# prachigarg23/MDIL-SS

Hardware: AMD Instinct MI355X
Metric: images/sec at 1024x512 ERFNet-RA step-2 train (CS->BDD, KD on), batch 6/GPU (higher is better)
Workload: dtype f32; 1 GPU; ERFNet-RAP step-2 (2 student fwd + teacher fwd + CE + 0.1*KLD + bwd + Adam), random-init weights of the reference architecture, num_classes [20,20]; batch_per_gpu=6, global_batch=6, height=512, width=1024, parallelism=dp1

## Files before the change

### include/mdil_hip.h

```cpp
#ifndef MDIL_HIP_H
#define MDIL_HIP_H

#include <stddef.h>

#ifdef __cplusplus
extern "C" {
#endif

#define MDIL_OK 0
#define MDIL_ERR_INVALID (-1)
#define MDIL_ERR_LAUNCH (-2)
#define MDIL_ERR_UNSUPPORTED (-3)

#define MDIL_MAX_TAPS 9

const char* mdil_last_error(void);
int mdil_version(void);

typedef struct mdil_geom {
  int N, HO, WO;
  int HI, WI;
  int ihs, iws;
  int ntaps;
  int dh[MDIL_MAX_TAPS], dw[MDIL_MAX_TAPS];
  int src[MDIL_MAX_TAPS];
  int in_pitch[2];
  int OH, OW;
  int ohs, oho, ows, owo;
  int out_pitch, out_coff;
} mdil_geom;

typedef struct mdil_epilogue {
  const float* bias;
  const float* scale;
  const float* shift;
  const float* res;
  const float* res_gate;
  const float* gate;
  int relu;
  const float* bias2;
} mdil_epilogue;

typedef struct mdil_pack_job {
  const float* src;
  float* dst;
  int ntaps, M, K, M_P, K_P, s_m, s_k, stem;
  int ktap[MDIL_MAX_TAPS];
} mdil_pack_job;
int mdil_pack_weights(const float* src, float* dst, int ntaps, const int* ktap, int M, int K,
                      int M_P, int K_P, int s_m, int s_k, int stem, void* stream);
int mdil_pack_weights_batch(const mdil_pack_job* jobs_device, int njobs, void* stream);

int mdil_tapconv(const mdil_geom* g, int cin, int cout, const float* in0, const float* in1,
                 const float* wpk, const mdil_epilogue* epi, float* out, void* stream);

int mdil_tapconv_stat_blocks(const mdil_geom* g, int cin, int cout);
int mdil_tapconv_stats(const mdil_geom* g, int cin, int cout, const float* in0, const float* in1,
                       const float* wpk, const mdil_epilogue* epi, float* out, float* partial,
                       float* pcount, void* stream);


typedef struct mdil_bn_train {
  const float *gamma, *beta;
  float *running_mean, *running_var;
  long long* num_batches_tracked;
  float eps, momentum;
  float* coef;
} mdil_bn_train;
int mdil_tapconv_bn_train(const mdil_geom* g, int cin, int cout, const float* in0, const float* in1,
                          const float* wpk, const mdil_epilogue* epi, float* out,
                          const mdil_bn_train* bn, void* workspace, size_t workspace_bytes,
                          unsigned int* ticket, void* stream);

typedef struct mdil_bn_grad {
  const float* gamma;
  float *dgamma, *dbeta;
  int accumulate;
  float* coef;
  unsigned int* ticket;
} mdil_bn_grad;

int mdil_tapconv_bnred(const mdil_geom* g, int cin, int cout, const float* in0, const float* in1,
                       const float* wpk, const mdil_epilogue* epi, float* out, const float* bn_z,
                       const float* save_mean, const float* save_invstd, float* partial,
                       const mdil_bn_grad* fin, void* stream);

typedef struct mdil_bn_tail {
  const float* gate;
  const float* z;
  const float* save_mean;
  const float* save_invstd;
  const float* drop;
  float* partial;
  mdil_bn_grad fin;
} mdil_bn_tail;
int mdil_tapconv_tail_blocks(const mdil_geom* g, int cin, int cout);
int mdil_tapconv_tail(const mdil_geom* g, int cin, int cout, const float* in0, const float* in1,
                      const float* wpk, const mdil_epilogue* epi, float* out, const mdil_bn_tail* tail,
                      void* stream);

size_t mdil_wgrad_workspace(const mdil_geom* g, int cin, int cout);
int mdil_wgrad(const mdil_geom* g, int cin, int cout, const float* in0, const float* in1,
               const float* gout, const int* ktap, int s_co, int s_ci, float* dw, float* dbias,
               int ntaps2, int s_co2, int s_ci2, float* dw2, float* dbias2,
               int accumulate ,
               void* workspace, size_t workspace_bytes, void* stream);

// ... 135 lines not shown
```

### mdil_ss_amd/_lib.py

```python
import ctypes as C
import os

_HERE = os.path.dirname(os.path.abspath(__file__))
LIB_PATH = os.environ.get("MDIL_HIP_LIB", os.path.join(_HERE, "libmdil_hip.so"))
MAX_TAPS = 9


class Geom(C.Structure):
    _fields_ = [("N", C.c_int), ("HO", C.c_int), ("WO", C.c_int), ("HI", C.c_int), ("WI", C.c_int),
                ("ihs", C.c_int), ("iws", C.c_int), ("ntaps", C.c_int),
                ("dh", C.c_int * MAX_TAPS), ("dw", C.c_int * MAX_TAPS), ("src", C.c_int * MAX_TAPS),
                ("in_pitch", C.c_int * 2), ("OH", C.c_int), ("OW", C.c_int),
                ("ohs", C.c_int), ("oho", C.c_int), ("ows", C.c_int), ("owo", C.c_int),
                ("out_pitch", C.c_int), ("out_coff", C.c_int)]


class PackJob(C.Structure):
    _fields_ = [("src", C.c_void_p), ("dst", C.c_void_p), ("ntaps", C.c_int), ("M", C.c_int),
                ("K", C.c_int), ("M_P", C.c_int), ("K_P", C.c_int), ("s_m", C.c_int),
                ("s_k", C.c_int), ("stem", C.c_int), ("ktap", C.c_int * MAX_TAPS)]


class Epilogue(C.Structure):
    _fields_ = [("bias", C.c_void_p), ("scale", C.c_void_p), ("shift", C.c_void_p),
# ... 8 lines not shown
        "dbeta")]


class BnGrad(C.Structure):
    _fields_ = [("gamma", C.c_void_p), ("dgamma", C.c_void_p), ("dbeta", C.c_void_p),
                ("accumulate", C.c_int), ("coef", C.c_void_p), ("ticket", C.c_void_p)]


class BnTrain(C.Structure):
    _fields_ = [("gamma", C.c_void_p), ("beta", C.c_void_p), ("running_mean", C.c_void_p),
                ("running_var", C.c_void_p), ("num_batches_tracked", C.c_void_p),
                ("eps", C.c_float), ("momentum", C.c_float), ("coef", C.c_void_p)]


class BnTail(C.Structure):
    _fields_ = [(n, C.c_void_p) for n in ("gate", "z", "save_mean", "save_invstd", "drop", "partial")] + \
               [("fin", BnGrad)]


class NbBlock(C.Structure):
    _fields_ = [("N", C.c_int), ("H", C.c_int), ("W", C.c_int), ("C", C.c_int),
                ("dilation", C.c_int), ("rap", C.c_int), ("train", C.c_int),
                ("bn_eps", C.c_float), ("bn_momentum", C.c_float), ("half", NbHalf * 2)] + \
               [(n, C.c_void_p) for n in ("x", "drop", "a1", "z1", "u", "a2", "z2", "out", "gy",
                                          "gz2", "ga", "gu", "gx")] + \
               [("bn_workspace", C.c_void_p), ("bn_workspace_bytes", C.c_size_t),
                ("wgrad_workspace", C.c_void_p), ("wgrad_workspace_bytes", C.c_size_t),
                ("head_partial", C.c_void_p), ("head_nblk", C.c_int), ("tail", BnTail),
                ("head_coef", C.c_void_p), ("ticket", C.c_void_p), ("eval_coef_ready", C.c_int)]


class WgradJob(C.Structure):
    _fields_ = [("opaque", C.c_ubyte * 192)]


class ProfileRecord(C.Structure):
    _fields_ = [("kind", C.c_int), ("path", C.c_int), ("cin", C.c_int), ("cout", C.c_int),
                ("ntaps", C.c_int), ("npix", C.c_longlong), ("ms", C.c_float)]


_P = C.c_void_p
_I = C.c_int
_L = C.c_longlong
_F = C.c_float
_D = C.c_double
_Z = C.c_size_t

_SIGNATURES = {
    "mdil_last_error": (C.c_char_p, []),
    "mdil_version": (_I, []),
    "mdil_pack_weights": (_I, [_P, _P, _I, C.POINTER(_I), _I, _I, _I, _I, _I, _I, _I, _P]),
    "mdil_pack_weights_batch": (_I, [_P, _I, _P]),
    "mdil_tapconv": (_I, [C.POINTER(Geom), _I, _I, _P, _P, _P, C.POINTER(Epilogue), _P, _P]),
    "mdil_tapconv_stat_blocks": (_I, [C.POINTER(Geom), _I, _I]),
    "mdil_tapconv_stats": (_I, [C.POINTER(Geom), _I, _I, _P, _P, _P, C.POINTER(Epilogue), _P, _P, _P, _P]),
    "mdil_tapconv_bnred": (_I, [C.POINTER(Geom), _I, _I, _P, _P, _P, C.POINTER(Epilogue), _P, _P, _P, _P,
                                _P, C.POINTER(BnGrad), _P]),
    "mdil_tapconv_bn_train": (_I, [C.POINTER(Geom), _I, _I, _P, _P, _P, C.POINTER(Epilogue), _P,
                                   C.POINTER(BnTrain), _P, _Z, _P, _P]),
    "mdil_bn_backward_apply": (_I, [_P, _P, _P, _L, _I, _I, _P, _P, _P, _P, _P]),
    "mdil_tapconv_tail_blocks": (_I, [C.POINTER(Geom), _I, _I]),
    "mdil_tapconv_tail": (_I, [C.POINTER(Geom), _I, _I, _P, _P, _P, C.POINTER(Epilogue), _P,
                               C.POINTER(BnTail), _P]),
    "mdil_nb_block_tail_blocks": (_I, [_I, _I, _I, _I, _I]),
    "mdil_bn_backward_partials": (_I, [_P, _P, _P, _L, _I, _I, _P, _P, _P, _P, _I, _P, _P, _I, _P, _P, _Z, _P]),
    "mdil_bn_train_finalize": (_I, [_P, _P, _I, _I, _P, _P, _P, _P, _P, _F, _F, _P, _P, _P, _P, _P]),
    "mdil_wgrad_workspace": (_Z, [C.POINTER(Geom), _I, _I]),
    "mdil_wgrad": (_I, [C.POINTER(Geom), _I, _I, _P, _P, _P, C.POINTER(_I), _I, _I, _P, _P,
                   _I, _I, _I, _P, _P, _I, _P, _Z, _P]),
    "mdil_bn_workspace": (_Z, [_L, _I]),
    "mdil_bn_train_stats": (_I, [_P, _L, _I, _P, _P, _P, _P, _P, _F, _F, _P, _P, _P, _P, _P, _Z, _P, _P]),
    "mdil_bn_eval_coeffs": (_I, [_I, _P, _P, _P, _P, _F, _P, _P, _P]),
    "mdil_bn_apply": (_I, [_P, _L, _I, _I, _P, _P, _P, _P, _I, _P, _P]),
    "mdil_bn_backward": (_I, [_P, _P, _P, _P, _L, _I, _I, _P, _P, _P, _P, _P, _I, _P, _P, _Z, _P, _P]),
    "mdil_maxpool_concat_fwd": (_I, [_P, _I, _I, _I, _I, _P, _I, _I, _P]),
    "mdil_maxpool_concat_bwd": (_I, [_P, _P, _I, _I, _I, _I, _I, _I, _P, _P]),
    "mdil_outconv_fwd": (_I, [_P, _P, _P, _I, _I, _I, _I, _I, _P, _P]),
    "mdil_nb_block_wgrad_workspace": (_Z, [_I, _I, _I, _I, _I, _I]),
    "mdil_nb_block_forward": (_I, [C.POINTER(NbBlock), _P]),
    "mdil_nb_block_backward": (_I, [C.POINTER(NbBlock), _P]),
    "mdil_nb_block_backward_deferred": (_I, [C.POINTER(NbBlock), C.POINTER(WgradJob), C.POINTER(_I),
                                             C.POINTER(_Z), _P]),
    "mdil_wgrad_deferred": (_I, [C.POINTER(Geom), _I, _I, _P, _P, _P, C.POINTER(_I), _I, _I, _P, _P,
                            _I, _I, _I, _P, _P, _P, _Z, C.POINTER(WgradJob), _P]),
    "mdil_wgrad_reduce_batch": (_I, [C.POINTER(WgradJob), _I, _P]),
    "mdil_head_workspace": (_Z, []),
    "mdil_head_ce": (_I, [_P, _P, _P, _I, _I, _I, _I, _P, _P, _P, _P, _P, _P, _P, _P, _I, _P, _P, _P, _Z, _P]),
    "mdil_head_kld": (_I, [_P, _P, _P, _P, _P, _P, _I, _I, _I, _I, _P, _P, _P, _P, _P, _I, _P, _Z, _P]),
    "mdil_loss_workspace": (_Z, [_L]),
    "mdil_ce_loss": (_I, [_P, _P, _P, _L, _I, _I, _P, _P, _P, _P, _P, _Z, _P]),
    "mdil_kld_loss": (_I, [_P, _P, _L, _I, _I, _P, _P, _P, _P, _Z, _P]),
    "mdil_argmax_confusion": (_I, [_P, _P, _L, _I, _I, _I, _P, _P, _P]),
    "mdil_adam_step": (_I, [_P, _P, _P, _P, _L, _D, _D, _D, _D, _D, _D, _D, _D, _P]),
    "mdil_augment_batch": (_I, [_P, _P, _P, _I, _I, _I, _I, _I, _P, _P, _P]),
    "mdil_nchw_to_nhwc": (_I, [_P, _I, _I, _I, _I, _P, _P]),
    "mdil_dropout_factors": (_I, [_P, _P, _P, _P, _I, _P]),
    "mdil_profile_begin": (_I, [_I]),
    "mdil_profile_end": (_I, [C.POINTER(ProfileRecord), _I]),
}

EXPORTS = tuple(_SIGNATURES)
_lib = None


def load():
    global _lib
# ... 21 lines not shown
```

### mdil_ss_amd/ops.py

```python
import ctypes as C
import weakref as _weakref

import torch

from . import _lib
from ._lib import Epilogue, Geom

BN_EPS = 1e-3
BN_MOMENTUM = 0.1


_raw_stream = torch._C._cuda_getCurrentRawStream
_cur_device = torch._C._cuda_getDevice


def _stream():
    return _raw_stream(_cur_device())


def _p(t):
    return None if t is None else t.data_ptr()


def _chk(t, name="tensor"):
# ... 563 lines not shown
    return gz


def bn_backward_partials(g, z, gamma, beta, coef, want_affine, partial, nblk, out=None):
    lib = _lib.load()
    Cc = z.shape[-1]
    npix = z.numel() // Cc
    gz = torch.empty_like(z) if out is None else out
    dg = db = None
    sunk = False
    if want_affine:
        sg, sb = _sink(gamma), _sink(beta)
        sunk = sg is not None and sb is not None
        if sunk:
            dg, db = sg, sb
        else:
            dgb = torch.zeros(2, Cc, dtype=torch.float32, device=z.device)
            dg, db = dgb[0], dgb[1]
    ws = _bn_ws(lib, npix, Cc, z.device)
    cws = ws.data_ptr() + (256 * 2 * Cc + 256) * 4
    _lib.check(lib.mdil_bn_backward_partials(_p(g), None, _p(z), npix, npix // z.shape[0], Cc, _p(gamma),
                                             coef.data_ptr(), coef.data_ptr() + 4 * Cc, partial, nblk,
                                             _p(dg), _p(db), 1, _p(gz), cws, 3 * Cc * 4, _stream()),
               "mdil_bn_backward_partials")
    if sunk or not want_affine:
        return gz, None, None
    return gz, dg, db


def _g_s1(N, H, W, Cc, taps, two_src=False):
    return make_geom(N, H, W, H, W, taps, Cc, H, W, Cc)


def _taps_3x1(d, flip=False):
    s = -1 if flip else 1
    return [(s * (k - 1) * d, 0, 0) for k in range(3)]


def _taps_1x3(d, flip=False):
    s = -1 if flip else 1
    return [(0, s * (k - 1) * d, 0) for k in range(3)]


_PAR = {0: [(1, 0)], 1: [(0, 1), (2, 0)]}


def _class_taps(a, b):
    taps, ktap = [], []
    for kh, dh in _PAR[a]:
        for kw, dw in _PAR[b]:
            taps.append((dh, dw, 0))
            ktap.append(kh * 3 + kw)
    return taps, ktap


class DownFn(torch.autograd.Function):

    @staticmethod
    def forward(ctx, x, w, b, gamma, beta, rm, rv, nbt, train, link_out):
        lib = _lib.load()
        ctx.sink_slot = SINK_SLOT
        ctx.link_out = link_out
        _chk(x, "x")
        N, H, W, cin = x.shape
        cc = w.shape[0]
        cout = cc + cin
        HO, WO = H // 2, W // 2
        stem = cin == 3
        z = torch.empty(N, HO, WO, cout, dtype=torch.float32, device=x.device)
        if stem:
            wp = _cached((w.data_ptr(), "stem"), lambda: pack_into(
                torch.empty(1, 16, 32, dtype=torch.float32, device=w.device), w, (0,), cc, 27,
                27, 1, stem=True), (w,))
            g = make_geom(N, HO, WO, H, W, [(0, 0, 0)], 3, HO, WO, cout, ihs=2, iws=2)
            tapconv(g, 27, cc, x, None, wp, z, bias=b)
        else:
            taps = [(kh - 1, kw - 1, 0) for kh in range(3) for kw in range(3)]
            g = make_geom(N, HO, WO, H, W, taps, cin, HO, WO, cout, ihs=2, iws=2)
            tapconv(g, cin, cc, x, None, pack_conv(w, "fwd"), z, bias=b)
        _lib.check(lib.mdil_maxpool_concat_fwd(_p(x), N, H, W, cin, _p(z), cout, cc, _stream()),
                   "mdil_maxpool_concat_fwd")
        if train:
            coef = bn_train_stats(z, gamma, beta, rm, rv, nbt)
            y = bn_apply(z, coef[2], coef[3], relu=True)
            ctx.save_for_backward(x, w, b, gamma, beta, z, y, coef)
            _log_gates(y)
            _attach_tail(link_out, y, z, coef, gamma, beta)
        else:
            ec = bn_eval_coeffs(gamma, beta, rm, rv)
            y = bn_apply(z, ec[0], ec[1], relu=True)
        ctx.stem = stem
        return y

    @staticmethod
    def backward(ctx, gy):
        global SINK_SLOT
        SINK_SLOT = ctx.sink_slot
        lib = _lib.load()
        x, w, b, gamma, beta, z, y, coef = ctx.saved_tensors
        gy = gy.contiguous()
        N, H, W, cin = x.shape
        cc = w.shape[0]
        cout = cc + cin
        HO, WO = H // 2, W // 2
        need = ctx.needs_input_grad
        gz, dgamma, dbeta = _bn_backward_maybe_fused(ctx.link_out, gy, y, z, gamma, beta, coef, need[3] or need[4])
        dw = db = gx = None
        if need[1] or need[2]:
            if ctx.stem:
                g = make_geom(N, HO, WO, H, W, [(0, 0, 0)], 3, HO, WO, cout, ihs=2, iws=2)
                dw, db = wgrad(g, 27, cc, x, None, gz, None, 0, 0, w, b)
            else:
                taps = [(kh - 1, kw - 1, 0) for kh in range(3) for kw in range(3)]
                g = make_geom(N, HO, WO, H, W, taps, cin, HO, WO, cout, ihs=2, iws=2)
                dw, db = wgrad(g, cin, cc, x, None, gz, tuple(range(9)), cin * 9, 9, w, b)
        if need[0]:
            gx = torch.empty_like(x)
            _lib.check(lib.mdil_maxpool_concat_bwd(_p(x), _p(gz), N, H, W, cin, cout, cc, _p(gx),
                                                   _stream()), "mdil_maxpool_concat_bwd")
            for a in (0, 1):
                for bb in (0, 1):
                    taps, ktap = _class_taps(a, bb)
                    g = make_geom(N, HO, WO, HO, WO, taps, cout, H, W, cin, ohs=2, oho=a, ows=2,
                                  owo=bb)
                    tapconv(g, cc, cin, gz, None, pack_conv(w, "dgrad", tuple(ktap)), gx, res=gx)
        return gx, dw, db, dgamma, dbeta, None, None, None, None, None


def _pack_pair_dgrad(w31, pw):
    if pw is None:
        return pack_conv(w31, "dgrad")
    Cc = w31.shape[0]

    def build():
        dst = torch.empty(4, Cc, Cc, dtype=torch.float32, device=w31.device)
        pack_into(dst[:3], w31, (0, 1, 2), Cc, Cc, 3, Cc * 3)
        pack_into(dst[3:], pw, (0,), Cc, Cc, 1, Cc)
        return dst

    return _cached((w31.data_ptr(), pw.data_ptr(), "pair_dgrad"), build, (w31, pw))


BLOCK_ABI = __import__("os").environ.get("MDIL_PY_BLOCKS") is None
_nb_ws_bytes = {}


DEFER_WGRAD = False
WGRAD_BATCH = int(__import__("os").environ.get("MDIL_WGRAD_BATCH", "16"))
WGRAD_ARENA_BYTES = WGRAD_BATCH * (20 << 20)


class _DeferState:
    __slots__ = ("jobs", "n", "cursor", "arena", "nout", "used")

    def __init__(self, device):
        self.jobs = (_lib.WgradJob * (WGRAD_BATCH + 4))()
        self.n = 0
        self.cursor = 0
        self.arena = torch.empty(WGRAD_ARENA_BYTES, dtype=torch.uint8, device=device)
        self.nout = C.c_int(0)
        self.used = C.c_size_t(0)


_defer_states = {}


def _defer_state(device):
    key = (_cur_device(), _raw_stream(_cur_device()))
    st = _defer_states.get(key)
    if st is None:
        if torch.cuda.is_current_stream_capturing():
            raise RuntimeError("mdil: the weight-gradient arena would be allocated during graph capture; "
                               "run one eager iteration on the same streams first")
        st = _defer_states[key] = _DeferState(device)
    return st


def flush_wgrad():
# ... 350 lines not shown
                    dw13, db13 = conv_wgrad(_taps_1x3(dil), a, gz, w13, b13)
                if pw is not None and npw:
                    dpw, dpb = conv_wgrad([(0, 0, 0)], inp, gz, pw, pb)
            G = make_geom(N, H, W, H, W, _taps_1x3(dil, flip=True), Cc, H, W, Cc)
            ga = tapconv(G, Cc, Cc, gz, None, pack_conv(w13, "dgrad"), torch.empty_like(gz), gate=a)
            if n31:
                dw31, db31 = conv_wgrad(_taps_3x1(dil), inp, ga, w31, b31)
            taps = _taps_3x1(dil, flip=True)
            wpk = _pack_pair_dgrad(w31, pw)
            if pw is not None:
                taps = taps + [(0, 0, 1)]
            G = make_geom(N, H, W, H, W, taps, Cc, H, W, Cc)
            fused = None
            if bnred is not None and res_in is None and not BN_BWD_UNFUSED:
                fused = tapconv_bnred(G, Cc, Cc, ga, gz, wpk, torch.empty_like(gz), *bnred)
            if fused is not None:
                ginp = fused
            else:
                ginp = tapconv(G, Cc, Cc, ga, gz, wpk, torch.empty_like(gz), res=res_in,
                               res_gate=res_gate)
            return ginp, dw31, db31, dw13, db13, dpw, dpb

        gz2, dg2, dbe2 = bn_backward(gy, out, drop, z2, g2, be2, c2, need[15] or need[16])
        gu, dw31_2, db31_2, dw13_2, db13_2, dpw2, dpb2 = pair_bwd(
            gz2, a2, u, w31_2, b31_2, w13_2, b13_2, pw2, pb2, ctx.dil, need[9] or need[10], need[11] or need[12],
            need[13] or need[14], None, None, bnred=(u, z1, c1))
        if isinstance(gu, tuple):
            g_, partial, nblk = gu
            gz1, dg1, dbe1 = bn_backward_partials(g_, z1, g1, be1, c1, need[7] or need[8], partial,
                                                  nblk, out=g_)
        else:
            gz1, dg1, dbe1 = bn_backward(gu, u, None, z1, g1, be1, c1, need[7] or need[8], out=gu)
        gx, dw31_1, db31_1, dw13_1, db13_1, dpw1, dpb1 = pair_bwd(
            gz1, a1, x, w31_1, b31_1, w13_1, b13_1, pw1, pb1, 1, need[1] or need[2], need[3] or need[4],
            need[5] or need[6], gy, out)
        res = [gx, dw31_1, db31_1, dw13_1, db13_1, dpw1, dpb1, dg1, dbe1,
               dw31_2, db31_2, dw13_2, db13_2, dpw2, dpb2, dg2, dbe2, None, None, None, None, None, None]
        for i in range(17):
            if not need[i]:
                res[i] = None
        return tuple(res)


class UpFn(torch.autograd.Function):

    @staticmethod
    def forward(ctx, x, w, b, gamma, beta, rm, rv, nbt, train, link_out):
        ctx.sink_slot = SINK_SLOT
        ctx.link_out = link_out
        _chk(x, "x")
        N, H, W, cin = x.shape
        cout = w.shape[1]
        z = torch.empty(N, 2 * H, 2 * W, cout, dtype=torch.float32, device=x.device)
        for a in (0, 1):
            for bb in (0, 1):
                taps, ktap = _class_taps(a, bb)
                g = make_geom(N, H, W, H, W, taps, cin, 2 * H, 2 * W, cout, ohs=2, oho=a, ows=2,
                              owo=bb)
                tapconv(g, cin, cout, x, None, pack_conv(w, "t_fwd", tuple(ktap)), z, bias=b)
        if train:
            coef = bn_train_stats(z, gamma, beta, rm, rv, nbt)
            y = bn_apply(z, coef[2], coef[3], relu=True)
            ctx.save_for_backward(x, w, b, gamma, beta, z, y, coef)
            _log_gates(y)
            _attach_tail(link_out, y, z, coef, gamma, beta)
        else:
            ec = bn_eval_coeffs(gamma, beta, rm, rv)
            y = bn_apply(z, ec[0], ec[1], relu=True, out=z)
        return y

    @staticmethod
    def backward(ctx, gy):
        global SINK_SLOT
        SINK_SLOT = ctx.sink_slot
        x, w, b, gamma, beta, z, y, coef = ctx.saved_tensors
        gy = gy.contiguous()
        N, H, W, cin = x.shape
        cout = w.shape[1]
        need = ctx.needs_input_grad
        gz, dgamma, dbeta = _bn_backward_maybe_fused(ctx.link_out, gy, y, z, gamma, beta, coef, need[3] or need[4])
        dw = db = gx = None
        if need[1] or need[2]:
            for a in (0, 1):
                for bb in (0, 1):
                    taps, ktap = _class_taps(a, bb)
                    g = make_geom(N, H, W, H, W, taps, cin, 2 * H, 2 * W, cout, ohs=2, oho=a, ows=2,
                                  owo=bb)
                    dw, db = wgrad(g, cin, cout, x, None, gz, tuple(ktap), 9, cout * 9, w, b, dw, db)
        if need[0]:
            taps = [(kh - 1, kw - 1, 0) for kh in range(3) for kw in range(3)]
            g = make_geom(N, H, W, 2 * H, 2 * W, taps, cout, H, W, cin, ihs=2, iws=2)
            gx = tapconv(g, cout, cin, gz, None, pack_conv(w, "t_dgrad"), torch.empty_like(x))
        return gx, dw, db, dgamma, dbeta, None, None, None, None, None


def _r4(v):
    return (v + 3) // 4 * 4


class OutFn(torch.autograd.Function):

    @staticmethod
    def forward(ctx, x, w, b):
        ctx.sink_slot = SINK_SLOT
        _chk(x, "x")
        N, H, W, cin = x.shape
        nc = w.shape[1]
        P = _r4(nc)
        y = torch.empty(N, 2 * H, 2 * W, P, dtype=torch.float32, device=x.device)
        if cin == 16 and w.is_contiguous() and b is not None:
            _lib.check(_lib.load().mdil_outconv_fwd(_p(x), _p(w), _p(b), N, H, W, nc, P, _p(y),
                                                    _stream()), "mdil_outconv_fwd")
# ... 346 lines not shown
```

Measured before the change: 271.6 images/sec.

## Merge four sub-pixel class convolutions into one kernel for upsample and downsample dgrad

Adds a HIP kernel that computes all four output parity classes of the stride-2 transposed-conv forward and the downsampler data-gradient in a single launch. Each input tile is loaded once and reused across the 3x3 taps, with MFMA accumulators for all four classes and interleaved output stores. The downsampler backward also folds the maxpool-concat gradient into the epilogue, which removes a separate kernel and the read-modify-write residual passes over gx. The cost is higher register and LDS pressure from keeping four accumulator sets, and only four fixed channel configurations are supported.

After: 274.3 images/sec (median of 6 runs). About the same (+1.0%).

```diff
diff --git a/include/mdil_hip.h b/include/mdil_hip.h
--- a/include/mdil_hip.h
+++ b/include/mdil_hip.h
@@ -53,6 +53,10 @@
 
 int mdil_tapconv(const mdil_geom* g, int cin, int cout, const float* in0, const float* in1,
                  const float* wpk, const mdil_epilogue* epi, float* out, void* stream);
+
+int mdil_tapconv_classes(int N, int H, int W, int cin, int cout, const float* in, int in_pitch,
+                         const float* wpk, const mdil_epilogue* epi, float* out, int out_pitch,
+                         const float* pool_x, int pool_coff, void* stream);
 
 int mdil_tapconv_stat_blocks(const mdil_geom* g, int cin, int cout);
 int mdil_tapconv_stats(const mdil_geom* g, int cin, int cout, const float* in0, const float* in1,
diff --git a/mdil_ss_amd/_lib.py b/mdil_ss_amd/_lib.py
--- a/mdil_ss_amd/_lib.py
+++ b/mdil_ss_amd/_lib.py
@@ -84,6 +84,7 @@
     "mdil_pack_weights": (_I, [_P, _P, _I, C.POINTER(_I), _I, _I, _I, _I, _I, _I, _I, _P]),
     "mdil_pack_weights_batch": (_I, [_P, _I, _P]),
     "mdil_tapconv": (_I, [C.POINTER(Geom), _I, _I, _P, _P, _P, C.POINTER(Epilogue), _P, _P]),
+    "mdil_tapconv_classes": (_I, [_I, _I, _I, _I, _I, _P, _I, _P, C.POINTER(Epilogue), _P, _I, _P, _I, _P]),
     "mdil_tapconv_stat_blocks": (_I, [C.POINTER(Geom), _I, _I]),
     "mdil_tapconv_stats": (_I, [C.POINTER(Geom), _I, _I, _P, _P, _P, C.POINTER(Epilogue), _P, _P, _P, _P]),
     "mdil_tapconv_bnred": (_I, [C.POINTER(Geom), _I, _I, _P, _P, _P, C.POINTER(Epilogue), _P, _P, _P, _P,
diff --git a/mdil_ss_amd/csrc/tapconv_classes.hip b/mdil_ss_amd/csrc/tapconv_classes.hip
--- /dev/null
+++ b/mdil_ss_amd/csrc/tapconv_classes.hip
@@ -0,0 +1,321 @@
+#include <type_traits>
+
+#include "common.h"
+
+namespace {
+
+constexpr int pos_dh(int p) { return p < 2 ? 1 : 0; }
+constexpr int pos_dw(int p) { return (p == 0 || p == 2) ? 1 : 0; }
+constexpr int pos_ntile(int p) { return p == 0 ? 1 : (p == 3 ? 4 : 2); }
+constexpr int pos_cls(int p, int j) { return p == 0 ? 3 : p == 1 ? (j == 0 ? 2 : 3) : p == 2 ? (j == 0 ? 1 : 3) : j; }
+constexpr int pos_tap(int p, int j) {
+  return p == 0 ? 0 : p == 1 ? (j == 0 ? 1 : 2) : p == 2 ? (j == 0 ? 3 : 6) : (j == 0 ? 4 : j == 1 ? 5 : j == 2 ? 7 : 8);
+}
+
+struct ClsArgs {
+  int N, H, W;
+  int in_pitch, out_pitch;
+  int pool_coff;
+  const float* in;
+  const float* wpk;
+  const float* pool_x;
+  float* out;
+};
+
+template <int CIN, int COUT, int BM_>
+struct ClsCfg {
+  static constexpr int BM = BM_;
+  static constexpr int KC = (CIN <= 48) ? CIN : 32;
+  static constexpr int NCHUNK = CIN / KC;
+  static constexpr int QPR = KC / 4;
+  static constexpr int LD = KC + 4;
+  static constexpr int MT = COUT / 16;
+  static constexpr int NT = BM / 16;
+  static constexpr bool SPLIT_CO = (MT % 4 == 0);
+  static constexpr int TM = SPLIT_CO ? MT / 4 : MT;
+  static constexpr int TN = SPLIT_CO ? NT : NT / 4;
+  static constexpr int IN_ITEMS = BM * QPR / MDIL_WG;
+  static constexpr int W_ITEMS = (COUT * QPR + MDIL_WG - 1) / MDIL_WG;
+  static constexpr int LDO = COUT + 4;
+  static constexpr int QO = COUT / 4;
+  static constexpr int SMEM_STAGE = (BM + 4 * COUT) * LD;
+  static constexpr int SMEM_OUT = 2 * BM * LDO + 2 * BM;
+  static constexpr int SMEM = SMEM_STAGE > SMEM_OUT ? SMEM_STAGE : SMEM_OUT;
+  static_assert(CIN % 16 == 0 && COUT % 16 == 0, "channel counts");
+  static_assert(CIN % KC == 0, "chunking");
+  static_assert((BM * QPR) % MDIL_WG == 0, "in-tile items");
+  static_assert(SPLIT_CO || (NT % 4 == 0), "pixel tiles per wave");
+  static_assert(MDIL_WG % QO == 0 && (BM * 2 * QO) % MDIL_WG == 0, "store loop");
+  static_assert(BM <= MDIL_WG, "output offsets");
+};
+
+template <int CIN, int COUT, int BM, bool POOL>
+__global__ __launch_bounds__(MDIL_WG) void tapconv_classes_kernel(const ClsArgs A, const mdil_epilogue e) {
+  using C = ClsCfg<CIN, COUT, BM>;
+  __shared__ __attribute__((aligned(16))) float smem[C::SMEM];
+  float* Is = smem;
+  float* Ws = smem + BM * C::LD;
+
+  const int tid = threadIdx.x;
+  const int lane = tid & 63, wave = tid >> 6;
+  const int li = lane & 15, lg = lane >> 4;
+  const int hw = A.H * A.W;
+  const int npix = A.N * hw;
+  const int tile0 = blockIdx.x * BM;
+
+  int it_i[C::IN_ITEMS], it_j[C::IN_ITEMS];
+  long long it_base[C::IN_ITEMS];
+#pragma unroll
+  for (int i = 0; i < C::IN_ITEMS; ++i) {
+    const int idx = tid + MDIL_WG * i;
+    const int P = tile0 + idx / C::QPR;
+    if (P < npix) {
+      const int r = P % hw;
+      it_i[i] = r / A.W;
+      it_j[i] = r - it_i[i] * A.W;
+      it_base[i] = (long long)P * A.in_pitch;
+    } else {
+      it_i[i] = 1 << 28;
+      it_j[i] = 0;
+      it_base[i] = 0;
+    }
+  }
+
+  f32x4 regI[C::IN_ITEMS];
+  f32x4 regW[4][C::W_ITEMS];
+  unsigned okI = 0;
+
+  auto issue_loads = [&](auto POS, int kc) {
+    constexpr int p = decltype(POS)::value;
+    constexpr int dh = pos_dh(p), dw = pos_dw(p);
+    const long long tap_off = ((long long)dh * A.W + dw) * A.in_pitch + kc * C::KC;
+#pragma unroll
+    for (int i = 0; i < C::IN_ITEMS; ++i) {
+      const int q = (tid + MDIL_WG * i) % C::QPR;
+      const bool ok = (it_i[i] + dh < A.H) && (it_j[i] + dw < A.W);
+      long long off = it_base[i] + (q * 4 + tap_off);
+      off = ok ? off : 0ll;
+      regI[i] = *reinterpret_cast<const f32x4*>(A.in + off);
+      okI = ok ? (okI | (1u << i)) : (okI & ~(1u << i));
+    }
+#pragma unroll
+    for (int j = 0; j < pos_ntile(p); ++j) {
+#pragma unroll
+      for (int i = 0; i < C::W_ITEMS; ++i) {
+        int idx = tid + MDIL_WG * i;
+        if constexpr ((COUT * C::QPR) % MDIL_WG != 0) idx = idx < COUT * C::QPR ? idx : 0;
+        const int co = idx / C::QPR, q = idx % C::QPR;
+        regW[j][i] = *reinterpret_cast<const f32x4*>(A.wpk + ((long long)(pos_tap(p, j) * COUT + co)) * CIN +
+                                                     kc * C::KC + q * 4);
+      }
+    }
+  };
+
+  auto write_lds = [&](auto POS) {
+    constexpr int p = decltype(POS)::value;
+#pragma unroll
+    for (int i = 0; i < C::IN_ITEMS; ++i) {
+      const int idx = tid + MDIL_WG * i;
+      const int px = idx / C::QPR, q = idx % C::QPR;
+      const f32x4 z = {0.f, 0.f, 0.f, 0.f};
+      *reinterpret_cast<f32x4*>(&Is[px * C::LD + q * 4]) = ((okI >> i) & 1u) ? regI[i] : z;
+    }
+#pragma unroll
+    for (int j = 0; j < pos_ntile(p); ++j) {
+#pragma unroll
+      for (int i = 0; i < C::W_ITEMS; ++i) {
+        const int idx = tid + MDIL_WG * i;
+        if (((COUT * C::QPR) % MDIL_WG == 0) || idx < COUT * C::QPR) {
+          const int co = idx / C::QPR, q = idx % C::QPR;
+          *reinterpret_cast<f32x4*>(&Ws[(j * COUT + co) * C::LD + q * 4]) = regW[j][i];
+        }
+      }
+    }
+  };
+
+  f32x4 acc[4][C::TM][C::TN];
+#pragma unroll
+  for (int c = 0; c < 4; ++c)
+#pragma unroll
+    for (int m = 0; m < C::TM; ++m)
+#pragma unroll
+      for (int n = 0; n < C::TN; ++n) acc[c][m][n] = f32x4{0.f, 0.f, 0.f, 0.f};
+
+  const int co_tile0 = C::SPLIT_CO ? wave * C::TM : 0;
+  const int px_tile0 = C::SPLIT_CO ? 0 : wave * C::TN;
+
+  auto mfma_stage = [&](auto POS) {
+    constexpr int p = decltype(POS)::value;
+#pragma unroll
+    for (int r = 0; r < C::KC / 16; ++r) {
+      f32x4 b[C::TN];
+#pragma unroll
+      for (int n = 0; n < C::TN; ++n)
+        b[n] = *reinterpret_cast<const f32x4*>(&Is[((px_tile0 + n) * 16 + li) * C::LD + r * 16 + lg * 4]);
+#pragma unroll
+      for (int j = 0; j < pos_ntile(p); ++j) {
+        f32x4 a[C::TM];
+#pragma unroll
+        for (int m = 0; m < C::TM; ++m)
+          a[m] = *reinterpret_cast<const f32x4*>(
+              &Ws[(j * COUT + (co_tile0 + m) * 16 + li) * C::LD + r * 16 + lg * 4]);
+#pragma unroll
+        for (int s = 0; s < 4; ++s)
+#pragma unroll
+          for (int m = 0; m < C::TM; ++m)
+#pragma unroll
+            for (int n = 0; n < C::TN; ++n)
+              acc[pos_cls(p, j)][m][n] = mfma16(a[m][s], b[n][s], acc[pos_cls(p, j)][m][n]);
+      }
+    }
+  };
+
+  auto position = [&](auto POS) {
+    constexpr int p = decltype(POS)::value;
+    for (int kc = 0; kc < C::NCHUNK; ++kc) {
+      __syncthreads();
+      write_lds(POS);
+      __syncthreads();
+      if (kc + 1 < C::NCHUNK) {
+        issue_loads(POS, kc + 1);
+      } else if constexpr (p < 3) {
+        issue_loads(std::integral_constant<int, p + 1>{}, 0);
+      }
+      __builtin_amdgcn_s_setprio(1);
+      mfma_stage(POS);
+      __builtin_amdgcn_s_setprio(0);
+    }
+  };
+  issue_loads(std::integral_constant<int, 0>{}, 0);
+  position(std::integral_constant<int, 0>{});
+  position(std::integral_constant<int, 1>{});
+  position(std::integral_constant<int, 2>{});
+  position(std::integral_constant<int, 3>{});
+
+  float* Os = smem;
+  long long* Ob = reinterpret_cast<long long*>(smem + 2 * BM * C::LDO);
+  const int OW = 2 * A.W;
+  const int q4 = (tid % C::QO) * 4;
+  f32x4 vscale = {1.f, 1.f, 1.f, 1.f}, vbias = {0.f, 0.f, 0.f, 0.f};
+  if (e.bias) vbias = *reinterpret_cast<const f32x4*>(e.bias + q4);
+  if (e.bias2) vbias += *reinterpret_cast<const f32x4*>(e.bias2 + q4);
+  if (e.scale) {
+    vscale = *reinterpret_cast<const f32x4*>(e.scale + q4);
+    vbias = vbias * vscale + *reinterpret_cast<const f32x4*>(e.shift + q4);
+  }
+#pragma unroll
+  for (int a = 0; a < 2; ++a) {
+    __syncthreads();
+#pragma unroll
+    for (int b = 0; b < 2; ++b)
+#pragma unroll
+      for (int n = 0; n < C::TN; ++n)
+#pragma unroll
+        for (int m = 0; m < C::TM; ++m)
+          *reinterpret_cast<f32x4*>(
+              &Os[(((px_tile0 + n) * 16 + li) * 2 + b) * C::LDO + (co_tile0 + m) * 16 + lg * 4]) =
+              acc[a * 2 + b][m][n];
+    if (a == 0 && tid < BM) {
+      const int P = tile0 + tid;
+      long long ob = -1;
+      if (P < npix) {
+        const int ni = P / hw;
+        const int r = P - ni * hw;
+        const int i = r / A.W;
+        const int j = r - i * A.W;
+        ob = ((long long)(ni * 2 * A.H + 2 * i) * OW + 2 * j) * A.out_pitch;
+      }
+      Ob[tid] = ob;
+    }
+    __syncthreads();
+    constexpr int NIT = BM * 2 * C::QO / MDIL_WG;
+#pragma unroll
+    for (int it = 0; it < NIT; ++it) {
+      const int idx = tid + it * MDIL_WG;
+      const int px = idx / (2 * C::QO);
+      const int b = (idx / C::QO) & 1;
+      const long long ob = Ob[px];
+      const bool ok = ob >= 0;
+      const long long obase = ok ? ob + ((long long)a * OW + b) * A.out_pitch + q4 : 0ll;
+      f32x4 v = *reinterpret_cast<const f32x4*>(&Os[(px * 2 + b) * C::LDO + q4]);
+      v = v * vscale + vbias;
+      if constexpr (POOL) {
+        const long long wb = ok ? ob + q4 : 0ll;
+        const long long down = (long long)OW * A.out_pitch;
+        const f32x4 x0 = *reinterpret_cast<const f32x4*>(A.pool_x + wb);
+        const f32x4 x1 = *reinterpret_cast<const f32x4*>(A.pool_x + wb + (ok ? A.out_pitch : 0));
+        const f32x4 x2 = *reinterpret_cast<const f32x4*>(A.pool_x + wb + (ok ? down : 0ll));
+        const f32x4 x3 = *reinterpret_cast<const f32x4*>(A.pool_x + wb + (ok ? down + A.out_pitch : 0ll));
+        const long long goff = ok ? (long long)(tile0 + px) * A.in_pitch + A.pool_coff + q4 : 0ll;
+        const f32x4 gg = *reinterpret_cast<const f32x4*>(A.in + goff);
+        f32x4 rr;
+#pragma unroll
+        for (int k = 0; k < 4; ++k) {
+          float m = x0[k];
+          int arg = 0;
+          if (x1[k] > m) { m = x1[k]; arg = 1; }
+          if (x2[k] > m) { m = x2[k]; arg = 2; }
+          if (x3[k] > m) { m = x3[k]; arg = 3; }
+          rr[k] = arg == a * 2 + b ? gg[k] : 0.f;
+        }
+        v += rr;
+      }
+      if (e.relu) {
+#pragma unroll
+        for (int k = 0; k < 4; ++k) v[k] = fmaxf(v[k], 0.f);
+      }
+      if (ok) __builtin_nontemporal_store(v, reinterpret_cast<f32x4*>(A.out + obase));
+    }
+  }
+}
+
+template <int CIN, int COUT, int BM>
+int launch_classes(const ClsArgs& a, const mdil_epilogue* epi, hipStream_t st) {
+  const long long npix = (long long)a.N * a.H * a.W;
+  const int grid = cdiv(npix, BM);
+  if (a.pool_x)
+    hipLaunchKernelGGL((tapconv_classes_kernel<CIN, COUT, BM, true>), dim3(grid), dim3(MDIL_WG), 0, st, a, *epi);
+  else
+    hipLaunchKernelGGL((tapconv_classes_kernel<CIN, COUT, BM, false>), dim3(grid), dim3(MDIL_WG), 0, st, a, *epi);
+  MDIL_CHECK_LAUNCH();
+  return MDIL_OK;
+}
+
+}
+
+extern "C" int mdil_tapconv_classes(int N, int H, int W, int cin, int cout, const float* in, int in_pitch,
+                                    const float* wpk, const mdil_epilogue* epi, float* out, int out_pitch,
+                                    const float* pool_x, int pool_coff, void* stream) {
+  MDIL_CHECK_ARG(in && wpk && epi && out, "tapconv_classes: null argument");
+  if (!((cin == 128 && cout == 64) || (cin == 64 && cout == 16) || (cin == 64 && cout == 64) ||
+        (cin == 48 && cout == 16))) {
+    mdil_set_error("tapconv_classes: no tile configuration for cin=%d cout=%d", cin, cout);
+    return MDIL_ERR_UNSUPPORTED;
+  }
+  MDIL_CHECK_ARG(N >= 1 && H >= 1 && W >= 1, "tapconv_classes: empty grid");
+  MDIL_CHECK_ARG((long long)N * H * W * 4 < (1ll << 31), "tapconv_classes: grid too large");
+  MDIL_CHECK_ARG(in_pitch >= cin && in_pitch % 4 == 0, "tapconv_classes: in_pitch=%d", in_pitch);
+  MDIL_CHECK_ARG(out_pitch >= cout && out_pitch % 4 == 0, "tapconv_classes: out_pitch=%d", out_pitch);
+  MDIL_CHECK_ARG((epi->scale == nullptr) == (epi->shift == nullptr), "tapconv_classes: scale/shift");
+  MDIL_CHECK_ARG(!epi->res && !epi->res_gate && !epi->gate, "tapconv_classes: residual / gate epilogues");
+  MDIL_CHECK_ARG(!pool_x || (pool_coff >= 0 && pool_coff % 4 == 0 && pool_coff + cout <= in_pitch),
+                 "tapconv_classes: pool_coff=%d", pool_coff);
+  ClsArgs a;
+  a.N = N, a.H = H, a.W = W;
+  a.in_pitch = in_pitch, a.out_pitch = out_pitch, a.pool_coff = pool_coff;
+  a.in = in, a.wpk = wpk, a.pool_x = pool_x, a.out = out;
+  hipStream_t st = (hipStream_t)stream;
+  mdil_geom g;
+  memset(&g, 0, sizeof(g));
+  g.N = N, g.HO = H, g.WO = W, g.ntaps = 9;
+  MdilProfScope ps(st, 0, &g, cin, cout);
+#define CL(ci, co, bm) \
+  if (cin == ci && cout == co) return launch_classes<ci, co, bm>(a, epi, st)
+  CL(128, 64, 64);
+  CL(64, 16, 128);
+  CL(64, 64, 64);
+  CL(48, 16, 128);
+#undef CL
+  mdil_set_error("tapconv_classes: no tile configuration for cin=%d cout=%d", cin, cout);
+  return MDIL_ERR_UNSUPPORTED;
+}
diff --git a/mdil_ss_amd/ops.py b/mdil_ss_amd/ops.py
--- a/mdil_ss_amd/ops.py
+++ b/mdil_ss_amd/ops.py
@@ -639,6 +639,19 @@
             taps.append((dh, dw, 0))
             ktap.append(kh * 3 + kw)
     return taps, ktap
+
+
+CLASS_MERGED = __import__("os").environ.get("MDIL_NO_CLSCONV") is None
+
+
+def tapconv_classes(x, cin, cout, wpk, out, bias=None, scale=None, shift=None, relu=False, pool_x=None,
+                    pool_coff=0):
+    N, H, W, pitch = x.shape
+    e = Epilogue(_p(bias), _p(scale), _p(shift), None, None, None, 1 if relu else 0, None)
+    _lib.check(_lib.load().mdil_tapconv_classes(N, H, W, cin, cout, _p(x), pitch, _p(wpk), C.byref(e),
+                                                _p(out), out.shape[3], _p(pool_x), pool_coff, _stream()),
+               "mdil_tapconv_classes")
+    return out
 
 
 class DownFn(torch.autograd.Function):
@@ -703,14 +716,17 @@
                 dw, db = wgrad(g, cin, cc, x, None, gz, tuple(range(9)), cin * 9, 9, w, b)
         if need[0]:
             gx = torch.empty_like(x)
-            _lib.check(lib.mdil_maxpool_concat_bwd(_p(x), _p(gz), N, H, W, cin, cout, cc, _p(gx),
-                                                   _stream()), "mdil_maxpool_concat_bwd")
-            for a in (0, 1):
-                for bb in (0, 1):
-                    taps, ktap = _class_taps(a, bb)
-                    g = make_geom(N, HO, WO, HO, WO, taps, cout, H, W, cin, ohs=2, oho=a, ows=2,
-                                  owo=bb)
-                    tapconv(g, cc, cin, gz, None, pack_conv(w, "dgrad", tuple(ktap)), gx, res=gx)
+            if CLASS_MERGED:
+                tapconv_classes(gz, cc, cin, pack_conv(w, "dgrad"), gx, pool_x=x, pool_coff=cc)
+            else:
+                _lib.check(lib.mdil_maxpool_concat_bwd(_p(x), _p(gz), N, H, W, cin, cout, cc, _p(gx),
+                                                       _stream()), "mdil_maxpool_concat_bwd")
+                for a in (0, 1):
+                    for bb in (0, 1):
+                        taps, ktap = _class_taps(a, bb)
+                        g = make_geom(N, HO, WO, HO, WO, taps, cout, H, W, cin, ohs=2, oho=a, ows=2,
+                                      owo=bb)
+                        tapconv(g, cc, cin, gz, None, pack_conv(w, "dgrad", tuple(ktap)), gx, res=gx)
         return gx, dw, db, dgamma, dbeta, None, None, None, None, None
 
 
@@ -1167,12 +1183,15 @@
         N, H, W, cin = x.shape
         cout = w.shape[1]
         z = torch.empty(N, 2 * H, 2 * W, cout, dtype=torch.float32, device=x.device)
-        for a in (0, 1):
-            for bb in (0, 1):
-                taps, ktap = _class_taps(a, bb)
-                g = make_geom(N, H, W, H, W, taps, cin, 2 * H, 2 * W, cout, ohs=2, oho=a, ows=2,
-                              owo=bb)
-                tapconv(g, cin, cout, x, None, pack_conv(w, "t_fwd", tuple(ktap)), z, bias=b)
+        if CLASS_MERGED:
+            tapconv_classes(x, cin, cout, pack_conv(w, "t_fwd"), z, bias=b)
+        else:
+            for a in (0, 1):
+                for bb in (0, 1):
+                    taps, ktap = _class_taps(a, bb)
+                    g = make_geom(N, H, W, H, W, taps, cin, 2 * H, 2 * W, cout, ohs=2, oho=a, ows=2,
+                                  owo=bb)
+                    tapconv(g, cin, cout, x, None, pack_conv(w, "t_fwd", tuple(ktap)), z, bias=b)
         if train:
             coef = bn_train_stats(z, gamma, beta, rm, rv, nbt)
             y = bn_apply(z, coef[2], coef[3], relu=True)
```

## Fuse four stride-2 parity-class tap convolutions into one kernel sharing input tiles

Applied to the files above, without the earlier changes.

Adds a HIP kernel that computes all four output parity classes of a stride-2 transposed convolution (upsample forward and downsample input-gradient) in a single launch. It loads one shared 2x2-shifted input tile into LDS and runs MFMA over all nine taps, instead of four separate tapconv launches that each re-read the input. It uses persistent work-groups capped at twice the CU count and falls back to the old path for uncovered shapes. Coverage is limited to a few specific channel configurations, and the fixed tiling may lower occupancy.

Measured after the change: 270.6 images/sec before, 271.4 images/sec after, median of 6. No clear change (+0.3%).

```diff
diff --git a/include/mdil_hip.h b/include/mdil_hip.h
--- a/include/mdil_hip.h
+++ b/include/mdil_hip.h
@@ -53,6 +53,10 @@
 
 int mdil_tapconv(const mdil_geom* g, int cin, int cout, const float* in0, const float* in1,
                  const float* wpk, const mdil_epilogue* epi, float* out, void* stream);
+
+int mdil_tapconv_s2x4_covers(const mdil_geom* g, int cin, int cout, const mdil_epilogue* epi);
+int mdil_tapconv_s2x4(const mdil_geom* g, int cin, int cout, const float* in0, const float* wpk9,
+                      const mdil_epilogue* epi, float* out, void* stream);
 
 int mdil_tapconv_stat_blocks(const mdil_geom* g, int cin, int cout);
 int mdil_tapconv_stats(const mdil_geom* g, int cin, int cout, const float* in0, const float* in1,
diff --git a/mdil_ss_amd/_lib.py b/mdil_ss_amd/_lib.py
--- a/mdil_ss_amd/_lib.py
+++ b/mdil_ss_amd/_lib.py
@@ -84,6 +84,8 @@
     "mdil_pack_weights": (_I, [_P, _P, _I, C.POINTER(_I), _I, _I, _I, _I, _I, _I, _I, _P]),
     "mdil_pack_weights_batch": (_I, [_P, _I, _P]),
     "mdil_tapconv": (_I, [C.POINTER(Geom), _I, _I, _P, _P, _P, C.POINTER(Epilogue), _P, _P]),
+    "mdil_tapconv_s2x4_covers": (_I, [C.POINTER(Geom), _I, _I, C.POINTER(Epilogue)]),
+    "mdil_tapconv_s2x4": (_I, [C.POINTER(Geom), _I, _I, _P, _P, C.POINTER(Epilogue), _P, _P]),
     "mdil_tapconv_stat_blocks": (_I, [C.POINTER(Geom), _I, _I]),
     "mdil_tapconv_stats": (_I, [C.POINTER(Geom), _I, _I, _P, _P, _P, C.POINTER(Epilogue), _P, _P, _P, _P]),
     "mdil_tapconv_bnred": (_I, [C.POINTER(Geom), _I, _I, _P, _P, _P, C.POINTER(Epilogue), _P, _P, _P, _P,
diff --git a/mdil_ss_amd/csrc/tapconv4.hip b/mdil_ss_amd/csrc/tapconv4.hip
--- /dev/null
+++ b/mdil_ss_amd/csrc/tapconv4.hip
@@ -0,0 +1,285 @@
+#include <stdlib.h>
+
+#include "common.h"
+
+namespace {
+
+__host__ __device__ constexpr int tap_cls(int t) { return t == 0 ? 0 : t < 3 ? 1 : t < 5 ? 2 : 3; }
+__host__ __device__ constexpr int tap_shift(int t) {
+  return (int)(((1u << 2 | 2u << 6 | 3u << 10 | 2u << 12 | 1u << 14) >> (2 * t)) & 3u);
+}
+
+template <int CIN, int COUT, int BM_, int KC_>
+struct X4Cfg {
+  static constexpr int BM = BM_, KC = KC_;
+  static constexpr int CIN_P = CIN;
+  static constexpr int NCH = CIN_P / KC;
+  static constexpr int QPR = KC / 4;
+  static constexpr int LD = KC + 4;
+  static constexpr int MT = COUT / 16, COUT_P = COUT;
+  static constexpr int NT = BM / 16;
+  static constexpr bool SPLIT_CO = (MT == 4);
+  static constexpr int TM = 1;
+  static constexpr int TN = SPLIT_CO ? NT : 1;
+  static constexpr int IN_ROWS = 4 * BM, W_ROWS = 9 * COUT_P;
+  static constexpr int IN_ITEMS = IN_ROWS * QPR / MDIL_WG;
+  static constexpr int W_ITEMS = (W_ROWS * QPR + MDIL_WG - 1) / MDIL_WG;
+  static constexpr bool W_RAGGED = (W_ROWS * QPR) % MDIL_WG != 0;
+  static constexpr int SMEM_STAGE = (IN_ROWS + W_ROWS) * LD;
+  static constexpr int LDO = COUT + 4;
+  static constexpr int SMEM_EPI_MAX = (NCH == 1) ? IN_ROWS * LD : SMEM_STAGE;
+  static constexpr int EPASS = (4 * BM * LDO + 2 * BM <= SMEM_EPI_MAX) ? 1 : 2;
+  static constexpr int CPP = 4 / EPASS;
+  static constexpr int QO = COUT / 4;
+  static constexpr int NIT = CPP * BM * QO / MDIL_WG;
+  static_assert(CIN % 16 == 0 && COUT % 16 == 0 && CIN_P % KC == 0 && KC % 16 == 0, "channels");
+  static_assert((IN_ROWS * QPR) % MDIL_WG == 0, "in-tile items");
+  static_assert(SPLIT_CO || (MT == 1 && NT == 2), "wave split");
+  static_assert(CPP * BM * LDO + 2 * BM <= SMEM_EPI_MAX, "epilogue staging");
+  static_assert((CPP * BM * QO) % MDIL_WG == 0 && MDIL_WG % QO == 0, "store items");
+  static_assert(SMEM_STAGE * 4 <= 80 * 1024, "two work-groups per CU");
+};
+
+template <int CIN, int COUT, int BM, int KC>
+__global__ __launch_bounds__(MDIL_WG) void tapconv4_kernel(const mdil_geom g, const float* __restrict__ in0,
+                                                           const float* __restrict__ wpk,
+                                                           const float* __restrict__ bias, const float* res,
+                                                           float* out) {
+  using C = X4Cfg<CIN, COUT, BM, KC>;
+  __shared__ __attribute__((aligned(16))) float smem[C::SMEM_STAGE];
+  float* Is = smem;
+  float* Ws = smem + C::IN_ROWS * C::LD;
+
+  const int tid = threadIdx.x;
+  const int lane = tid & 63;
+  const int wave = __builtin_amdgcn_readfirstlane(tid >> 6);
+  const int li = lane & 15, lg = lane >> 4;
+  const int npix = g.N * g.HO * g.WO;
+  const int hw = g.HO * g.WO;
+  const int pitch = g.in_pitch[0];
+  const int ntile = (npix + BM - 1) / BM;
+  const int my_tiles = ((int)blockIdx.x < ntile) ? (ntile - 1 - (int)blockIdx.x) / (int)gridDim.x + 1 : 0;
+  const int nstage = my_tiles * C::NCH;
+
+  const int co_tile0 = C::SPLIT_CO ? wave : 0;
+  const int px_tile0 = C::SPLIT_CO ? 0 : (wave & 1);
+  const unsigned cls_mask = C::SPLIT_CO ? 0xFu : ((wave >> 1) ? 0x6u : 0x9u);
+
+  long long it_off[C::IN_ITEMS];
+  f32x4 regI[C::IN_ITEMS];
+  f32x4 regW[C::W_ITEMS];
+
+  auto issue_loads = [&](int st) {
+    const int tile = blockIdx.x + (st / C::NCH) * gridDim.x;
+    const int kc = st % C::NCH;
+    if (kc == 0) {
+#pragma unroll
+      for (int i = 0; i < C::IN_ITEMS; ++i) {
+        const int row = (tid + MDIL_WG * i) / C::QPR;
+        const int s = row / BM, p = row % BM;
+        const int P = tile * BM + p;
+        long long off = -1;
+        if (P < npix) {
+          const int n = P / hw;
+          const int r = P - n * hw;
+          const int h = r / g.WO;
+          const int hi = h + (s >> 1), wi = r - h * g.WO + (s & 1);
+          if (hi < g.HI && wi < g.WI) off = (((long long)n * g.HI + hi) * g.WI + wi) * pitch;
+        }
+        it_off[i] = off;
+      }
+    }
+#pragma unroll
+    for (int i = 0; i < C::IN_ITEMS; ++i) {
+      const int q = (tid + MDIL_WG * i) % C::QPR;
+      const long long off = it_off[i] < 0 ? 0ll : it_off[i];
+      regI[i] = *reinterpret_cast<const f32x4*>(in0 + off + kc * KC + q * 4);
+    }
+    if (C::NCH > 1 || st == 0) {
+#pragma unroll
+      for (int i = 0; i < C::W_ITEMS; ++i) {
+        int idx = tid + MDIL_WG * i;
+        if constexpr (C::W_RAGGED) idx = idx < C::W_ROWS * C::QPR ? idx : 0;
+        const int row = idx / C::QPR, q = idx % C::QPR;
+        regW[i] = *reinterpret_cast<const f32x4*>(wpk + (long long)row * C::CIN_P + kc * KC + q * 4);
+      }
+    }
+  };
+
+  auto write_lds = [&](int st) {
+#pragma unroll
+    for (int i = 0; i < C::IN_ITEMS; ++i) {
+      const int idx = tid + MDIL_WG * i;
+      const int row = idx / C::QPR, q = idx % C::QPR;
+      const f32x4 z = {0.f, 0.f, 0.f, 0.f};
+      *reinterpret_cast<f32x4*>(&Is[row * C::LD + q * 4]) = it_off[i] < 0 ? z : regI[i];
+    }
+    if (C::NCH > 1 || st == 0) {
+#pragma unroll
+      for (int i = 0; i < C::W_ITEMS; ++i) {
+        const int idx = tid + MDIL_WG * i;
+        if (!C::W_RAGGED || idx < C::W_ROWS * C::QPR) {
+          const int row = idx / C::QPR, q = idx % C::QPR;
+          *reinterpret_cast<f32x4*>(&Ws[row * C::LD + q * 4]) = regW[i];
+        }
+      }
+    }
+  };
+
+  f32x4 acc[4][C::TN];
+  auto zero_acc = [&]() {
+#pragma unroll
+    for (int c = 0; c < 4; ++c)
+#pragma unroll
+      for (int n = 0; n < C::TN; ++n) acc[c][n] = f32x4{0.f, 0.f, 0.f, 0.f};
+  };
+  zero_acc();
+
+  f32x4 vbias = {0.f, 0.f, 0.f, 0.f};
+  if (bias) vbias = *reinterpret_cast<const f32x4*>(bias + (tid % C::QO) * 4);
+
+  auto epilogue = [&](int tile) {
+    float* Os = smem;
+    long long* Ob = reinterpret_cast<long long*>(smem + C::CPP * BM * C::LDO);
+#pragma unroll
+    for (int pass = 0; pass < C::EPASS; ++pass) {
+      __syncthreads();
+#pragma unroll
+      for (int c = 0; c < C::CPP; ++c) {
+        const int cls = pass * C::CPP + c;
+        if ((cls_mask >> cls) & 1u) {
+          const int a_local = c >> 1, b = c & 1;
+#pragma unroll
+          for (int n = 0; n < C::TN; ++n) {
+            const int p = (px_tile0 + n) * 16 + li;
+            *reinterpret_cast<f32x4*>(&Os[((a_local * BM + p) * 2 + b) * C::LDO + co_tile0 * 16 + lg * 4]) =
+                acc[cls][n];
+          }
+        }
+      }
+      if (pass == 0 && tid < BM) {
+        const int P = tile * BM + tid;
+        long long ob = -1;
+        if (P < npix) {
+          const int n = P / hw;
+          const int r = P - n * hw;
+          const int h = r / g.WO;
+          const int w = r - h * g.WO;
+          ob = (((long long)n * g.OH + 2 * h) * g.OW + 2 * w) * g.out_pitch + g.out_coff;
+        }
+        Ob[tid] = ob;
+      }
+      __syncthreads();
+#pragma unroll
+      for (int it = 0; it < C::NIT; ++it) {
+        const int idx = tid + it * MDIL_WG;
+        const int row = idx / C::QO, q = idx % C::QO;
+        const int b = row & 1, p = (row >> 1) % BM;
+        const int a = (C::EPASS == 2) ? pass : (row >> 1) / BM;
+        const long long ob = Ob[p];
+        const bool ok = ob >= 0;
+        const long long o = (ok ? ob : 0ll) + ((long long)a * g.OW + b) * g.out_pitch + q * 4;
+        f32x4 v = *reinterpret_cast<const f32x4*>(&Os[row * C::LDO + q * 4]);
+        v = v + vbias;
+        if (res) v += *reinterpret_cast<const f32x4*>(res + (ok ? o : 0ll));
+        if (ok) __builtin_nontemporal_store(v, reinterpret_cast<f32x4*>(out + o));
+      }
+    }
+  };
+
+  if (nstage > 0) issue_loads(0);
+  for (int st = 0; st < nstage; ++st) {
+    __syncthreads();
+    write_lds(st);
+    __syncthreads();
+    if (st + 1 < nstage) issue_loads(st + 1);
+    __builtin_amdgcn_s_setprio(1);
+#pragma unroll
+    for (int t = 0; t < 9; ++t) {
+      const int cls = tap_cls(t), sh = tap_shift(t);
+      if ((cls_mask >> cls) & 1u) {
+#pragma unroll
+        for (int r = 0; r < KC / 16; ++r) {
+          f32x4 b[C::TN];
+          const f32x4 a =
+              *reinterpret_cast<const f32x4*>(&Ws[((t * C::MT + co_tile0) * 16 + li) * C::LD + r * 16 + lg * 4]);
+#pragma unroll
+          for (int n = 0; n < C::TN; ++n)
+            b[n] = *reinterpret_cast<const f32x4*>(
+                &Is[(sh * BM + (px_tile0 + n) * 16 + li) * C::LD + r * 16 + lg * 4]);
+#pragma unroll
+          for (int s = 0; s < 4; ++s)
+#pragma unroll
+            for (int n = 0; n < C::TN; ++n) acc[cls][n] = mfma16(a[s], b[n][s], acc[cls][n]);
+        }
+      }
+    }
+    __builtin_amdgcn_s_setprio(0);
+    if (st % C::NCH == C::NCH - 1) {
+      epilogue(blockIdx.x + (st / C::NCH) * gridDim.x);
+      zero_acc();
+    }
+  }
+}
+
+int x4_num_cu() {
+  static int n_cu = 0;
+  if (n_cu == 0) {
+    int dev = 0, n = 0;
+    if (hipGetDevice(&dev) != hipSuccess ||
+        hipDeviceGetAttribute(&n, hipDeviceAttributeMultiprocessorCount, dev) != hipSuccess || n <= 0)
+      n = 256;
+    n_cu = n;
+  }
+  return n_cu;
+}
+
+template <int CIN, int COUT, int BM, int KC>
+int launch_x4(const mdil_geom* g, const float* in0, const float* wpk, const mdil_epilogue* epi, float* out,
+              hipStream_t st) {
+  const long long npix = (long long)g->N * g->HO * g->WO;
+  const int ntile = cdiv(npix, BM);
+  const int cap = 2 * x4_num_cu();
+  const int grid = ntile < cap ? ntile : cap;
+  hipLaunchKernelGGL((tapconv4_kernel<CIN, COUT, BM, KC>), dim3(grid), dim3(MDIL_WG), 0, st, *g, in0, wpk,
+                     epi->bias, epi->res, out);
+  MDIL_CHECK_LAUNCH();
+  return MDIL_OK;
+}
+
+}
+
+extern "C" int mdil_tapconv_s2x4_covers(const mdil_geom* g, int cin, int cout, const mdil_epilogue* epi) {
+  static const bool on = getenv("MDIL_NO_S2X4") == nullptr;
+  if (!on || !g || !epi) return 0;
+  if (epi->scale || epi->shift || epi->res_gate || epi->gate || epi->relu || epi->bias2) return 0;
+  int pitch;
+  if (cin == 128 && cout == 64) pitch = 128;
+  else if (cin == 64 && cout == 16) pitch = 64;
+  else if (cin == 48 && cout == 16) pitch = 64;
+  else return 0;
+  if (g->in_pitch[0] != pitch || g->ntaps != 9) return 0;
+  if (g->N < 1 || g->HO < 1 || g->WO < 1 || g->HI != g->HO || g->WI != g->WO) return 0;
+  if (g->ihs != 1 || g->iws != 1 || g->ohs != 2 || g->ows != 2 || g->oho != 0 || g->owo != 0) return 0;
+  if (g->OH != 2 * g->HO || g->OW != 2 * g->WO) return 0;
+  if (g->out_pitch % 4 != 0 || g->out_coff % 4 != 0 || g->out_coff < 0 || g->out_coff + cout > g->out_pitch)
+    return 0;
+  if ((long long)g->N * g->HO * g->WO >= (1ll << 31) - 64) return 0;
+  for (int t = 0; t < 9; ++t)
+    if (g->src[t] != 0 || g->dh[t] != (tap_shift(t) >> 1) || g->dw[t] != (tap_shift(t) & 1)) return 0;
+  return 1;
+}
+
+extern "C" int mdil_tapconv_s2x4(const mdil_geom* g, int cin, int cout, const float* in0, const float* wpk9,
+                                 const mdil_epilogue* epi, float* out, void* stream) {
+  MDIL_CHECK_ARG(g && epi && in0 && wpk9 && out, "tapconv_s2x4: null argument");
+  if (!mdil_tapconv_s2x4_covers(g, cin, cout, epi)) {
+    mdil_set_error("tapconv_s2x4: call is not covered (cin=%d cout=%d)", cin, cout);
+    return MDIL_ERR_UNSUPPORTED;
+  }
+  hipStream_t st = (hipStream_t)stream;
+  MdilProfScope ps(st, 0, g, cin, cout);
+  if (cin == 128) return launch_x4<128, 64, 64, 16>(g, in0, wpk9, epi, out, st);
+  if (cin == 64) return launch_x4<64, 16, 32, 64>(g, in0, wpk9, epi, out, st);
+  return launch_x4<48, 16, 32, 48>(g, in0, wpk9, epi, out, st);
+}
diff --git a/mdil_ss_amd/ops.py b/mdil_ss_amd/ops.py
--- a/mdil_ss_amd/ops.py
+++ b/mdil_ss_amd/ops.py
@@ -639,6 +639,28 @@
             taps.append((dh, dw, 0))
             ktap.append(kh * 3 + kw)
     return taps, ktap
+
+
+_S2X4_TAPS, _S2X4_KTAP = [], []
+for _a in (0, 1):
+    for _b in (0, 1):
+        _t, _k = _class_taps(_a, _b)
+        _S2X4_TAPS += _t
+        _S2X4_KTAP += _k
+_S2X4_KTAP = tuple(_S2X4_KTAP)
+
+
+def tapconv_s2x4(N, H, W, in_pitch, cin, cout, out_pitch, inp, w, mode, out, bias=None, res=None,
+                 OH=None, OW=None):
+    lib = _lib.load()
+    g = make_geom(N, H, W, H, W, _S2X4_TAPS, in_pitch, 2 * H if OH is None else OH,
+                  2 * W if OW is None else OW, out_pitch, ohs=2, ows=2)
+    e = Epilogue(_p(bias), None, None, _p(res), None, None, 0, None)
+    if not lib.mdil_tapconv_s2x4_covers(C.byref(g), cin, cout, C.byref(e)):
+        return False
+    _lib.check(lib.mdil_tapconv_s2x4(C.byref(g), cin, cout, _p(inp), _p(pack_conv(w, mode, _S2X4_KTAP)),
+                                     C.byref(e), _p(out), _stream()), "mdil_tapconv_s2x4")
+    return True
 
 
 class DownFn(torch.autograd.Function):
@@ -705,12 +727,13 @@
             gx = torch.empty_like(x)
             _lib.check(lib.mdil_maxpool_concat_bwd(_p(x), _p(gz), N, H, W, cin, cout, cc, _p(gx),
                                                    _stream()), "mdil_maxpool_concat_bwd")
-            for a in (0, 1):
-                for bb in (0, 1):
-                    taps, ktap = _class_taps(a, bb)
-                    g = make_geom(N, HO, WO, HO, WO, taps, cout, H, W, cin, ohs=2, oho=a, ows=2,
-                                  owo=bb)
-                    tapconv(g, cc, cin, gz, None, pack_conv(w, "dgrad", tuple(ktap)), gx, res=gx)
+            if not tapconv_s2x4(N, HO, WO, cout, cc, cin, cin, gz, w, "dgrad", gx, res=gx, OH=H, OW=W):
+                for a in (0, 1):
+                    for bb in (0, 1):
+                        taps, ktap = _class_taps(a, bb)
+                        g = make_geom(N, HO, WO, HO, WO, taps, cout, H, W, cin, ohs=2, oho=a, ows=2,
+                                      owo=bb)
+                        tapconv(g, cc, cin, gz, None, pack_conv(w, "dgrad", tuple(ktap)), gx, res=gx)
         return gx, dw, db, dgamma, dbeta, None, None, None, None, None
 
 
@@ -1167,12 +1190,13 @@
         N, H, W, cin = x.shape
         cout = w.shape[1]
         z = torch.empty(N, 2 * H, 2 * W, cout, dtype=torch.float32, device=x.device)
-        for a in (0, 1):
-            for bb in (0, 1):
-                taps, ktap = _class_taps(a, bb)
-                g = make_geom(N, H, W, H, W, taps, cin, 2 * H, 2 * W, cout, ohs=2, oho=a, ows=2,
-                              owo=bb)
-                tapconv(g, cin, cout, x, None, pack_conv(w, "t_fwd", tuple(ktap)), z, bias=b)
+        if not tapconv_s2x4(N, H, W, cin, cin, cout, cout, x, w, "t_fwd", z, bias=b):
+            for a in (0, 1):
+                for bb in (0, 1):
+                    taps, ktap = _class_taps(a, bb)
+                    g = make_geom(N, H, W, H, W, taps, cin, 2 * H, 2 * W, cout, ohs=2, oho=a, ows=2,
+                                  owo=bb)
+                    tapconv(g, cin, cout, x, None, pack_conv(w, "t_fwd", tuple(ktap)), z, bias=b)
         if train:
             coef = bn_train_stats(z, gamma, beta, rm, rv, nbt)
             y = bn_apply(z, coef[2], coef[3], relu=True)
```
